# DavidRother/cooking_zoo

Hardware: AMD Instinct MI355X
Metric: env-steps/sec at N parallel envs (1/2/4/8 GPU) + achieved HBM GB/s (higher is better)
Workload: dtype u8/u32 state, f64 obs+reward

## Files before the change

cooking_zoo_amd/csrc/cz_device.h:

```cpp
#pragma once
#include <hip/hip_runtime.h>
#include <stdint.h>
#include <type_traits>

namespace cz {

constexpr int MAX_AGENTS = 4;
constexpr int MAX_NODES = 8;
constexpr int WIDE_NODES = 16;
constexpr int HDR_WORDS = 8;
constexpr int AGENT_WORD0 = HDR_WORDS;
constexpr int RET_WORD0 = HDR_WORDS + MAX_AGENTS;
constexpr int CELL_WORD0 = RET_WORD0 + 2 * MAX_AGENTS;

enum : uint32_t { FLOOR = 0, COUNTER, DELIVERSQUARE, SWITCH, BLOCK, CUTBOARD, BLENDER };
enum : uint32_t { PLATE = 0, ONION, TOMATO, LETTUCE, CARROT, CUCUMBER, BANANA, APPLE, WATERMELON, BREAD };
enum : uint32_t { CELL_TYPE = 7, CELL_READY = 8, CELL_TOGGLE = 16, CELL_ACTIVE = 32, CELL_WALK = 64 };
enum : uint32_t { D_ALIVE = 1u << 24, D_CHOPPED = 2u << 24, D_MASHED = 4u << 24, D_FREE = 8u << 24, D_DONE = 6u << 24 };
enum : uint32_t { COND_NONE = 0, COND_CHOPPED, COND_MASHED, COND_NOT_CHOPPED, COND_NOT_MASHED };
enum : uint32_t { W_T = 0, W_MARKS, W_LAYOUT, W_STATUS, W_EPISODE, W_RECIPES, W_POOL, W_MARKS_HI };
enum : uint32_t { ST_DONE = 1, ST_TERM = 2, ST_TRUNC = 4 };
constexpr int LUT_Y0 = 63, LUT_ZERO = 126, LUT_ONE = 127;
constexpr int LUT_NDONE0 = 128, LUT_CH0 = 132, LUT_MA0 = 136, LUT_CF0 = 140, LUT_OR0 = 144;
enum : uint32_t { SU_EPISODES = 0, SU_STEPS, SU_LENSUM, SU_TRUNC, SU_TERM, SU_COMPLETED0, SU_LAST_LENGTH = 9, SU_LAST_EPISODE, SU_LAST_FLAGS,
// ... 14 lines not shown
    union {
        uint8_t *codes;
        float *obs32;
    };
    uint32_t *stat_u;
    double *stat_f;
    int64_t env_id_base;
    uint64_t seed;
    double recipe_reward, recipe_penalty, node_reward, time_penalty_step;
    double reward_idle;
    const double *lut;
    int32_t N, A, W, H, D, F, RW, scheme, max_steps, end_all, R, auto_reset, L;
    int32_t T;
    uint32_t step0;
    int32_t dyn0_off, dyn1_off;
    int32_t wt;
    int32_t walk_touches;
    int32_t wide;
#ifdef CZ_PROFILE
    unsigned long long *stamps;
#endif
#ifdef CZ_TIMELINE
    unsigned long long *timeline;
#endif
};
#if !defined(CZ_TIMELINE) && !defined(CZ_PROFILE)
static_assert(sizeof(Params) <= 264 && sizeof(Params) % 8 == 0, "argument block: see the note above");
#endif

struct LeanParams {
    const uint32_t *recipes;
    const uint32_t *lay_desc;
    int32_t L, F;
    int32_t max_steps;
    uint32_t settings;
    double reward_idle;
    double *rewards;
    uint8_t *term, *trunc;
    double *obs;
    int32_t auto_reset;
    int32_t reserved;
    uint32_t *stat_u;
    double *stat_f;
    const uint32_t *lay_init;
    int64_t env_id_base;
    double node_reward, recipe_reward, recipe_penalty, time_penalty_step;
#ifdef CZ_PROFILE
    unsigned long long *stamps;
#endif
#ifdef CZ_TIMELINE
    unsigned long long *timeline;
#endif
};
constexpr int LEADING_SCALAR_BYTES = 56;
#if !defined(CZ_TIMELINE) && !defined(CZ_PROFILE)
static_assert(LEADING_SCALAR_BYTES + sizeof(LeanParams) <= 4 * 64, "the lean argument block: four 64-byte lines with the leading scalars");
#endif
static_assert(LEADING_SCALAR_BYTES + offsetof(LeanParams, obs) + sizeof(double *) == 2 * 64, "the common path's fields end the second line");
struct LeanView : LeanParams {
    uint32_t *state;
    const int32_t *actions;
    const double *lut;
    int32_t N, RW, W, H, D, dyn0_off, dyn1_off;
    static constexpr int32_t wide = 0, wt = 1, T = 1;
    static constexpr uint32_t step0 = 0u;
    static constexpr uint64_t seed = 0u;
    static constexpr uint8_t *codes = nullptr;
    int32_t R, end_all, walk_touches;
    LeanView() = default;
    __host__ __device__ explicit LeanView(const LeanParams &b)
        : LeanParams(b), R((int32_t)(b.settings & 0xFFu)), end_all((int32_t)((b.settings >> 8) & 1u)), walk_touches((int32_t)((b.settings >> 16) & 1u)) {}
};
template <int R_, int END_ALL, int WALK_TOUCHES>
struct LeanViewFixed : LeanView {
    static_assert(R_ >= 1 && R_ <= 4 && (END_ALL | 1) == 1 && (WALK_TOUCHES | 1) == 1, "no such handle");
    static constexpr int32_t R = R_, end_all = END_ALL, walk_touches = WALK_TOUCHES;
    using LeanView::LeanView;
};
template <class PB> using block_of = std::conditional_t<std::is_base_of<LeanParams, PB>::value, LeanParams, Params>;

#ifndef CZ_PRIO
#define CZ_PRIO 1
#endif
#if CZ_PRIO
#define CZ_SETPRIO(p) __builtin_amdgcn_s_setprio(p)
#else
#define CZ_SETPRIO(p) do { } while (0)
#endif
__device__ __forceinline__ uint32_t rfl(uint32_t v) { return __builtin_amdgcn_readfirstlane(v); }
__device__ __forceinline__ uint32_t rdl(uint32_t v, int l) { return __builtin_amdgcn_readlane(v, l); }
__device__ __forceinline__ uint64_t ballot(bool p) { return __builtin_amdgcn_ballot_w64(p); }
__device__ __forceinline__ bool lanes(uint64_t m) { return __builtin_amdgcn_inverse_ballot_w64(m); }
extern "C" __device__ uint32_t __cz_writelane(uint32_t, uint32_t, uint32_t) __asm("llvm.amdgcn.writelane.i32");
__device__ __forceinline__ uint32_t wrl(uint32_t value, int lane, uint32_t into) { return __cz_writelane(value, (uint32_t)lane, into); }

__host__ __device__ inline uint32_t action_hash(uint64_t seed, int64_t env_global, int agent, uint32_t step, uint32_t n) {
    uint32_t x = (uint32_t)seed ^ ((uint32_t)(seed >> 32) * 0x9E3779B1u);
    x ^= (uint32_t)env_global * 0x85EBCA6Bu + (uint32_t)((uint64_t)env_global >> 32) * 0x27D4EB2Fu;
    x ^= ((uint32_t)agent + 1u) * 0xC2B2AE35u;
    x ^= (step + 1u) * 0x165667B1u;
    x ^= x >> 16; x *= 0x7FEB352Du; x ^= x >> 15; x *= 0x846CA68Bu; x ^= x >> 16;
    x += step * 0x9E3779B9u;
    x ^= x >> 16; x *= 0x7FEB352Du; x ^= x >> 15; x *= 0x846CA68Bu; x ^= x >> 16;
    return (uint32_t)(((uint64_t)x * (uint64_t)n) >> 32);
}
__host__ __device__ inline uint32_t next_layout(int64_t env_global, uint32_t episode, uint32_t pool_word, uint32_t n_layouts,
                                                uint32_t groups = 1u, uint32_t active = 0u) {
    uint32_t base = pool_word & 0xFFFFu, count = pool_word >> 16;
    if (count == 0) { base = 0; count = n_layouts; }
    if (groups > 1u) { count /= groups; base += active * count; }
    return base + (uint32_t)(((uint64_t)env_global + (uint64_t)episode * 7919u) % count);
}
constexpr int LAY_CTL_WORDS = 16;
enum : uint32_t { LC_GROUPS = 0, LC_ACTIVE = 1 };

struct SpawnCfg {
    uint64_t seed;
    double despawn_rate, respawn_rate;
    uint32_t grace_period;
    uint32_t stride;
    const uint8_t *areas;
    const uint8_t *level_of_layout;
    uint32_t *exhausted;
};
static_assert(sizeof(SpawnCfg) == 56, "layout of the block behind Params::lut");
constexpr uint32_t SPAWN_CFG_OFFSET = 256 * 8 + 64 * 4;
constexpr uint32_t COORD_TABLE_OFFSET = SPAWN_CFG_OFFSET + 56, ROWSEL_TABLE_OFFSET = COORD_TABLE_OFFSET + 1024 * 4;
constexpr uint32_t LUT_BLOCK_BYTES = ROWSEL_TABLE_OFFSET + 64 * 4;
constexpr int SPAWN_GONE0 = 8, SPAWN_GRACE0 = 12;
__host__ __device__ inline uint32_t spawn_grace_bits(uint32_t grace_period, int n_agents) { return grace_period <= 31u ? 5u : 20u / (uint32_t)n_agents; }
__host__ __device__ inline uint32_t spawn_max_grace(int n_agents) { const uint32_t b = 20u / (uint32_t)n_agents; return b > 5u ? (1u << b) - 1u : 31u; }
__host__ __device__ inline uint32_t spawn_initial_status(uint32_t packed_grace, int n_agents) {
    const uint32_t grace = packed_grace & 0xFFFFFFu, bits = packed_grace >> 24;
    uint32_t st = 0;
    for (int a = 0; a < n_agents; ++a) st |= grace << (SPAWN_GRACE0 + bits * a);
    return st;
}

enum : uint32_t { HDR_LAYOUT = 1u, HDR_RECIPE = 2u, HDR_POOL = 4u };
__host__ __device__ inline uint32_t record_header_faults(uint32_t layout, uint32_t recipes, uint32_t pool, uint32_t L, int R, uint32_t n_recipes) {
    uint32_t faults = layout < L ? 0u : HDR_LAYOUT;
    for (int k = 0; k < R; ++k)
        if (((recipes >> (8 * k)) & 0xFFu) >= n_recipes) faults |= HDR_RECIPE;
    const uint32_t base = pool & 0xFFFFu, count = pool >> 16;
    if (count && base + count > L) faults |= HDR_POOL;
    return faults;
}
__host__ __device__ inline bool slot_dead_but_tagged(uint32_t d0, uint32_t d1) { return !(d0 & D_ALIVE) && (d1 & 0xFFu); }

__host__ __device__ inline uint64_t spawn_mix(uint64_t x) {
    x = (x ^ (x >> 30)) * 0xBF58476D1CE4E5B9ull;
    x = (x ^ (x >> 27)) * 0x94D049BB133111EBull;
    return x ^ (x >> 31);
}
__host__ __device__ inline double spawn_uniform(uint64_t seed, uint64_t env_global, uint64_t step_key, uint32_t agent, uint32_t draw) {
    uint64_t k = spawn_mix(seed + 0x9E3779B97F4A7C15ull * env_global);
    k = spawn_mix(k ^ (step_key * 0xD1B54A32D192ED03ull));
    k = spawn_mix(k ^ ((uint64_t)agent << 32) ^ (uint64_t)draw);
    return (double)(k >> 11) * (1.0 / 9007199254740992.0);
}

template <int N>
struct Mask {
    uint64_t w[N];
    __device__ __forceinline__ bool any() const {
        uint64_t o = 0;
// ... 250 lines not shown
                const OM fr = dyn & m_d0_any(e, D_FREE);
                const int grab = fr.any() ? fr.first() : dyn.last();
                if (direct.test(grab)) {
                    me.h = grab;
                    touch(dt, slot_d0(e, grab));
                    move_obj(e, cx, grab, me.xy);
                }
            }
        } else {
            dt.interacted = 1;
            attempt_merge(e, cx, me, dyn, lxy, c, sv, dt);
        }
    }

    static __device__ __forceinline__ void pick_up_special(E &e, const Ctx &cx, Me &me, const OM &dyn, Dirty &dt) {
        if (me.h >= 0 || !dyn.any()) return;
        const OM plates = dyn & m_d0(e, 0xFF0000u, PLATE << 16);
        if (plates.count() != 1) return;
        const int p = plates.first();
        const OM cm = content_of(e, p);
        const int cnt = cm.count();
        if (cnt == 0) return;
        const OM lastm = cm & m_d1(e, 0xFF00u, (uint32_t)(cnt - 1) << 8);
        const int s = lastm.first();
#pragma unroll
        for (int k = 0; k < OPL; ++k) {
            const bool mine = (cx.lane + 64 * k) == s;
            e.d1[k] = mine ? 0u : e.d1[k];
        }
        me.h = s;
        touch(dt, slot_d0(e, s));
        move_obj(e, cx, s, me.xy);
        dt.interacted = 1;
    }

    static __device__ __forceinline__ void execute(E &e, const Ctx &cx, uint32_t lxy, int c, uint32_t sv, const OM &dyn, Dirty &dt) {
        const uint32_t ty = sv & CELL_TYPE;
        if (ty == CUTBOARD) {
            if (!(sv & CELL_READY)) return;
            const OM fresh = dyn & outside_plates(e) & m_d0(e, D_CHOPPED, 0u);
            const int f = fresh.first();
            if (f < 0) return;
            const uint32_t fw = slot_d0(e, f);
            slot_or(e, cx, f, D_CHOPPED);
            if ((fw & 0xFF0000u) == (BREAD << 16)) {
                const OM spare = m_d0(e, D_ALIVE | 0xFF0000u, BREAD << 16);
                const int n = spare.first();
#pragma unroll
                for (int k = 0; k < OPL; ++k) {
                    const bool mine = (cx.lane + 64 * k) == n;
                    e.d0[k] = mine ? (lxy | (BREAD << 16) | D_ALIVE | D_CHOPPED | D_FREE) : e.d0[k];
                    e.d1[k] = mine ? 0u : e.d1[k];
                }
            }
            cell_update(e, cx, c, CELL_READY, 0, dt);
            touch_change(dt, fw, fw | D_CHOPPED);
            dt.interacted = 1;
        } else if (ty == BLENDER) {
            if (sv & CELL_READY) cell_update(e, cx, c, 0, CELL_TOGGLE, dt);
        }
    }

    static __device__ __forceinline__ bool cell_bit(const CM &m, uint32_t c) {
        if constexpr (CPL == 1) {
            return ((m.w[0] >> (c & 63u)) & 1ull) != 0ull;
        } else {
            uint32_t hit = 0u;
#pragma unroll
            for (int k = 0; k < CPL; ++k) {
                const uint32_t lo = (uint32_t)m.w[k], hi = (uint32_t)(m.w[k] >> 32);
                const uint32_t half = (c & 32u) ? hi : lo;
                hit |= ((c >> 6) == (uint32_t)k) ? (half >> (c & 31u)) : 0u;
            }
            return (hit & 1u) != 0u;
        }
    }
    template <int CTRL>
    static __device__ __forceinline__ uint32_t quad(uint32_t v) {
        return (uint32_t)__builtin_amdgcn_mov_dpp((int)v, CTRL, 0xF, 0xF, true);
    }

    struct Pre { uint64_t inter; uint32_t txy, c, act; };

    static __device__ __forceinline__ void perform_agent_actions(E &e, const Ctx &cx, uint32_t act_raw, Dirty &dt) {
        const Pre pre = agents_walk(e, cx, act_raw, dt);
        agents_interact(e, cx, pre, dt);
    }

    static __device__ __forceinline__ Pre agents_walk(E &e, const Ctx &cx, uint32_t act_raw, Dirty &dt) {
        const uint32_t W = (uint32_t)cx.W, H = (uint32_t)cx.H;
        const uint64_t present_m = ~(uint64_t)((e.status >> SPAWN_GONE0) & 0xFu);
        const uint32_t agw = e.agw;
        const uint32_t x = agw & 0xFFu, y = (agw >> 8) & 0xFFu, xy = agw & 0xFFFFu;
        const uint64_t agent_m = ballot((int32_t)act_raw >= 0) & ((1ull << NA) - 1ull) & present_m;
        const uint32_t act0 = lanes(agent_m) ? (act_raw & 7u) : 0u;
        const uint32_t sh = 2u * act0;
        const uint32_t tx = x + ((DX_TABLE >> sh) & 3u) - 1u, ty = y + ((DY_TABLE >> sh) & 3u) - 1u;
        uint32_t ag = lanes(ballot(act0 - 1u < 4u)) ? ((agw & 0xFF00FFFFu) | (act0 << 16)) : agw;
        const uint64_t inb_m = ballot(tx < W) & ballot(ty < H);
        const uint32_t own = __umul24(y, W) + x;
        uint32_t txy = lanes(inb_m) ? (tx | (ty << 8)) : xy;
        uint32_t c = lanes(inb_m) ? (__umul24(ty, W) + tx) : own;
        uint64_t moving_m = ballot(act0 != 0u) & inb_m;
        CM walk_set, switch_set;
#pragma unroll
        for (int k = 0; k < CPL; ++k) {
            walk_set.w[k] = ballot(walkable(e.cell[k]));
            switch_set.w[k] = ballot((e.cell[k] & CELL_TYPE) == SWITCH);
        }
        const uint64_t wk_m = ballot(cell_bit(walk_set, c));
        if (NA > 1) {
            const uint32_t endxy = lanes(wk_m) ? txy : xy;
            const uint32_t exy = lanes(agent_m) ? endxy : (0xFFFF0000u | (uint32_t)cx.lane);
            uint64_t clash_m;
            if (NA == 2) {
                clash_m = ballot(exy == quad<0xB1>(exy));
            } else {
                const uint32_t r1 = quad<0x39>(exy), r2 = quad<0x4E>(exy), r3 = quad<0x93>(exy);
                clash_m = ballot(exy == r1) | ballot(exy == r2) | ballot(exy == r3);
            }
            const uint64_t cancel_m = clash_m & wk_m & moving_m;
            txy = lanes(cancel_m) ? xy : txy;
            c = lanes(cancel_m) ? own : c;
            moving_m &= ~cancel_m;
        }
        const uint32_t act = lanes(moving_m) ? act0 : 0u;
        uint64_t walks_m = agent_m & wk_m;
        if (SCHEME != 3) walks_m &= ballot(act - 1u < 4u);
        ag = lanes(walks_m) ? ((ag & 0xFFFF0000u) | txy) : ag;
        e.agw = ag;
        uint64_t drag = walks_m & moving_m & ballot(ag > 0x00FFFFFFu);
        if (drag) {
            dt.moved = 1;
            do {
                const int a = __builtin_ctzll(drag);
                drag &= drag - 1;
                const uint32_t A = rdl(e.agw, a);
                move_obj(e, cx, (int)(A >> 24) - 1, A & 0xFFFFu);
            } while (drag);
        }
        uint64_t press = walks_m & ballot(cell_bit(switch_set, c));
        if (press) {
            dt.pressed = 1;
            do {
                const int a = __builtin_ctzll(press);
                press &= press - 1;
                cell_update(e, cx, (int)rdl(c, a), 0, CELL_ACTIVE, dt);
            } while (press);
        }
        return Pre{agent_m & ~walks_m & (SCHEME == 3 ? moving_m : ballot(act >= 5u)), txy, c, act};
    }

    static __device__ __forceinline__ void agents_interact(E &e, const Ctx &cx, const Pre &pre, Dirty &dt) {
        const uint32_t W = (uint32_t)cx.W, H = (uint32_t)cx.H;
        const uint32_t txy = pre.txy, c = pre.c, act = pre.act;
        uint64_t inter = pre.inter;
        if (inter & (inter - 1)) CZ_SETPRIO(2);
        else if (inter) CZ_SETPRIO(1);
#ifndef CZ_INTER_UNROLL
#define CZ_INTER_UNROLL 0
#endif
#if CZ_INTER_UNROLL
#pragma unroll
        for (int a = 0; a < NA; ++a) {
            if (!((inter >> a) & 1ull)) continue;
#else
        while (inter) {
            const int a = __builtin_ctzll(inter);
            inter &= inter - 1;
#endif
            const uint32_t A = rdl(e.agw, a);
            Me me{A & 0xFFFFu, (int)(A >> 24) - 1};
            uint32_t fxy;
            int fc;
            bool ok = true;
            if (SCHEME == 3) {
                fxy = rdl(txy, a);
                fc = (int)rdl(c, a);
            } else {
                const uint32_t o = (A >> 16) & 0xFFu;
                const uint32_t fx = (A & 0xFFu) + ((DX_TABLE >> (2u * o)) & 3u) - 1u;
                const uint32_t fy = ((A >> 8) & 0xFFu) + ((DY_TABLE >> (2u * o)) & 3u) - 1u;
                ok = fx < W && fy < H;
                fxy = fx | (fy << 8);
                fc = (int)(fy * W + fx);
            }
            const uint32_t sv = ok ? cell_at(e, fc) : 0u;
            if (ok && holds_objects(sv & CELL_TYPE)) {
                const OM dyn = m_d0(e, D_ALIVE | 0xFFFFu, D_ALIVE | fxy);
                if (SCHEME == 3) {
                    bool exec = false;
                    if ((sv & CELL_TYPE) >= CUTBOARD) exec = (dyn & m_d0(e, D_DONE, 0u)).any();
                    if (exec) execute(e, cx, fxy, fc, sv, dyn, dt);
                    else primary(e, cx, me, fxy, fc, sv, dyn, dt);
                } else {
                    const int ac = (int)rdl(act, a);
                    if (ac == 5) primary(e, cx, me, fxy, fc, sv, dyn, dt);
                    else if (ac == 6) pick_up_special(e, cx, me, dyn, dt);
                    else execute(e, cx, fxy, fc, sv, dyn, dt);
                }
                e.agw = wrl((A & 0x00FFFFFFu) | ((uint32_t)((me.h + 1) & 0xFF) << 24), a, e.agw);
            }
        }
    }

    static __device__ __forceinline__ uint32_t handle_agent_spawn(E &e, const Ctx &cx, const SpawnCfg *cfg_generic, int64_t env_global) {
        typedef const __attribute__((address_space(4))) SpawnCfg *kcfg;
        const kcfg cfg = (kcfg)cfg_generic;
        const uint64_t seed = cfg->seed, key = ((uint64_t)e.episode << 32) | (uint64_t)e.t;
        const double despawn_rate = cfg->despawn_rate, respawn_rate = cfg->respawn_rate;
        uint32_t st = e.status, gone = 0u;
        const uint32_t packed_grace = cfg->grace_period, gbits = packed_grace >> 24, gmask = (1u << gbits) - 1u;
#pragma unroll
        for (int a = 0; a < NA; ++a) {
            const uint32_t gsh = (uint32_t)SPAWN_GRACE0 + gbits * (uint32_t)a;
            if ((st >> gsh) & gmask) { st -= 1u << gsh; continue; }
            const bool despawned = (st >> (SPAWN_GONE0 + a)) & 1u;
            if (!despawned) {
                const int n_active = NA - __popc((st >> SPAWN_GONE0) & 0xFu);
                if (n_active > 1 && spawn_uniform(seed, (uint64_t)env_global, key, (uint32_t)a, 0u) < despawn_rate) {
                    if ((rdl(e.agw, a) >> 24) == 0u) {
                        st |= 1u << (SPAWN_GONE0 + a);
                        gone |= 1u << a;
                    }
                }
            } else if (spawn_uniform(seed, (uint64_t)env_global, key, (uint32_t)a, 1u) < respawn_rate) {
                st = (st & ~(1u << (SPAWN_GONE0 + a))) | ((packed_grace & 0xFFFFFFu) << gsh);
                typedef const __attribute__((address_space(4))) uint8_t *kbytes;
                const uint32_t stride = cfg->stride, level = ((kbytes)cfg->level_of_layout)[e.layout];
                const kbytes blk = (kbytes)cfg->areas + (size_t)(level * (uint32_t)MAX_AGENTS + (uint32_t)a) * (4u + 2u * stride);
                const uint32_t nx = (uint32_t)blk[0] | ((uint32_t)blk[1] << 8), ny = (uint32_t)blk[2] | ((uint32_t)blk[3] << 8);
                bool placed = false;
#pragma nounroll
                for (uint32_t k = 0; k < 1001u; ++k) {
                    const uint32_t ix = (uint32_t)(spawn_uniform(seed, (uint64_t)env_global, key, (uint32_t)a, 2u + 2u * k) * (double)nx);
                    const uint32_t iy = (uint32_t)(spawn_uniform(seed, (uint64_t)env_global, key, (uint32_t)a, 3u + 2u * k) * (double)ny);
                    const uint32_t x = blk[4u + ix], y = blk[4u + stride + iy];
                    if (x >= (uint32_t)cx.W || y >= (uint32_t)cx.H) continue;
                    if ((cell_at(e, (int)(y * (uint32_t)cx.W + x)) & CELL_TYPE) != FLOOR) continue;
// ... 305 lines not shown
```

cooking_zoo_amd/csrc/cz_kernels.h:

```cpp
#pragma once
#include "cz_device.h"
#include <type_traits>

namespace cz {

#ifdef CZ_PROFILE
#define CZ_STAMP(i)                                                                                    \
    do {                                                                                               \
        unsigned long long _t;                                                                         \
        __builtin_amdgcn_sched_barrier(0);                                                             \
        asm volatile("s_memrealtime %0\n\ts_waitcnt lgkmcnt(0)" : "=s"(_t)::"memory");                 \
        __builtin_amdgcn_sched_barrier(0);                                                             \
        if (lane == 0 && P.stamps) P.stamps[(size_t)env * 16 + (i)] = _t;                               \
    } while (0)
#elif defined(CZ_MARKERS)
#define CZ_STAMP(i) asm volatile("; CZ_MARK " #i)
#else
#define CZ_STAMP(i) do { } while (0)
#endif

typedef const __attribute__((address_space(4))) Params *KParams;
struct StepArgsMirror { uint32_t *a; const int32_t *b; const double *c; int32_t i[8]; Params p; };
struct LeanArgsMirror { uint32_t *a; const int32_t *b; const double *c; int32_t i[8]; LeanParams p; };
static_assert(offsetof(LeanArgsMirror, p) == LEADING_SCALAR_BYTES && offsetof(StepArgsMirror, p) == LEADING_SCALAR_BYTES, "leading scalars");
template <class B> constexpr unsigned block_offset() {
    return std::is_same<B, LeanParams>::value ? (unsigned)offsetof(LeanArgsMirror, p) : (unsigned)offsetof(StepArgsMirror, p);
}
template <class B = Params>
__device__ __forceinline__ const __attribute__((address_space(4))) B *late_params(unsigned offset) {
    const __attribute__((address_space(4))) char *k =
        (const __attribute__((address_space(4))) char *)__builtin_amdgcn_kernarg_segment_ptr();
    asm volatile("" : "+s"(k));
    return reinterpret_cast<const __attribute__((address_space(4))) B *>(k + offset);
}
#define CZ_LATE_STEP() late_params<typename V::Block>(block_offset<typename V::Block>())

enum StepMode : int {
    STEP = 0,
    ROLLOUT = 1,
    ROLLOUT_ACTIONS = 2,
    STEP_CODES = 3,
    ROLLOUT_CODES = 4,
    ROLLOUT_CODES_ONLY = 5,
    STEP_F32 = 6,
    ROLLOUT_F32 = 7,
    ROLLOUT_ACTIONS_F32 = 8,
};
template <int MODE, bool LEAN = false>
struct StepTraits {
    static_assert(MODE >= STEP && MODE <= ROLLOUT_ACTIONS_F32 && (!LEAN || MODE == STEP), "no such variant");
    static constexpr bool fused = MODE == ROLLOUT || MODE == ROLLOUT_ACTIONS || MODE == ROLLOUT_CODES || MODE == ROLLOUT_CODES_ONLY ||
                                  MODE == ROLLOUT_F32 || MODE == ROLLOUT_ACTIONS_F32;
    static constexpr bool ext_actions = MODE == ROLLOUT_ACTIONS || MODE == ROLLOUT_ACTIONS_F32;
    static constexpr bool codes = MODE == STEP_CODES || MODE == ROLLOUT_CODES || MODE == ROLLOUT_CODES_ONLY;
    static constexpr bool codes_only = MODE == ROLLOUT_CODES_ONLY;
    static constexpr bool f32 = MODE == STEP_F32 || MODE == ROLLOUT_F32 || MODE == ROLLOUT_ACTIONS_F32;
    static constexpr bool f64 = !codes_only && !f32;
#ifndef CZ_ROLLOUT_F32_HOLD
#define CZ_ROLLOUT_F32_HOLD 1
#endif
    static constexpr bool desc_held = (codes || f32) && (!fused || codes_only || (f32 && CZ_ROLLOUT_F32_HOLD != 0));
    static constexpr bool desc_per_step = (codes || f32) && fused && !desc_held;
    static constexpr bool lean = LEAN;
    using Block = std::conditional_t<LEAN, LeanParams, Params>;
    using View = std::conditional_t<LEAN, LeanView, Params>;
};
template <int R, int END_ALL, int WALK_TOUCHES>
struct LeanCfgTraits : StepTraits<STEP, true> {
    using View = LeanViewFixed<R, END_ALL, WALK_TOUCHES>;
};

template <int CPL>
struct Img {
    static constexpr bool HUGE = CPL > 4;
    static constexpr int OBJ0 = 0, CELL0 = HUGE ? 1536 : 768, AG0 = CELL0 + (HUGE ? 4096 : 1024), ZERO = AG0 + 32, HALFWORDS = ZERO + 8;
};
constexpr int LUT_ABSENT = 255, LUT_SIZE = 256;
#ifndef CZ_ENVS_PER_WG
#define CZ_ENVS_PER_WG 8
#endif
constexpr int ENVS_PER_WG = CZ_ENVS_PER_WG;
template <int CPL> constexpr int envs_per_wg() { return CPL > 4 ? 4 : ENVS_PER_WG; }
constexpr int OBS_PAIRS = 3;
constexpr int OBS_CHUNK = 2 * OBS_PAIRS;

template <int CPL>
struct Lds {
    int32_t sub[MAX_AGENTS][16];
    uint16_t img[Img<CPL>::HALFWORDS];
    uint64_t locs[CPL <= 4 ? 64 * CPL + 8 : WIDE_NODES * CPL];
};

template <class T>
__device__ __forceinline__ T ldg(const void *sbase, uint32_t voff) {
    return *reinterpret_cast<const T *>(reinterpret_cast<const char *>(sbase) + voff);
}
template <class T>
__device__ __forceinline__ void stg(void *sbase, uint32_t voff, T v) {
    *reinterpret_cast<T *>(reinterpret_cast<char *>(sbase) + voff) = v;
}
template <class T>
__device__ __forceinline__ void stg_wt(void *sbase, uint32_t voff, T v) {
    __hip_atomic_store(reinterpret_cast<T *>(reinterpret_cast<char *>(sbase) + voff), v, __ATOMIC_RELAXED, __HIP_MEMORY_SCOPE_AGENT);
}

typedef double double2_t __attribute__((ext_vector_type(2)));
typedef uint32_t uint2_t __attribute__((ext_vector_type(2)));
typedef uint32_t uint4_t __attribute__((ext_vector_type(4)));

template <int OPL, int CPL, int NA, bool LEAN = false, class PB>
__device__ __forceinline__ void load_env(const PB &P, Env<OPL, CPL, NA> &e, const Ctx &cx, const uint32_t *__restrict__ rec) {
    const uint32_t lane = (uint32_t)cx.lane;
    uint32_t hw[HDR_WORDS];
    {
        typedef const __attribute__((address_space(4))) uint32_t *kconst_u32;
        const kconst_u32 hp = (kconst_u32)rec;
#pragma unroll
        for (int i = 0; i < HDR_WORDS; ++i) hw[i] = hp[i];
    }
    const uint32_t aw = ldg<uint32_t>(rec, (AGENT_WORD0 + (lane & 3u)) * 4u);
#pragma unroll
    for (int k = 0; k < CPL; ++k) {
        const uint32_t c = lane + 64u * k;
        const uint32_t v = ldg<uint8_t>(rec, CELL_WORD0 * 4u + min(c, (uint32_t)cx.C - 1u));
        e.cell[k] = (c < (uint32_t)cx.C) ? v : 0u;
    }
#pragma unroll
    for (int k = 0; k < OPL; ++k) {
        const uint32_t s = lane + 64u * k, sc = min(s, (uint32_t)cx.D - 1u);
        const uint32_t a = ldg<uint32_t>(rec, ((uint32_t)P.dyn0_off + sc) * 4u), b = ldg<uint32_t>(rec, ((uint32_t)P.dyn1_off + sc) * 4u);
        e.d0[k] = (s < (uint32_t)cx.D) ? a : 0u;
        e.d1[k] = (s < (uint32_t)cx.D) ? b : 0u;
    }
    __builtin_amdgcn_sched_barrier(0);
    e.t = hw[W_T]; e.marks = hw[W_MARKS]; e.layout = hw[W_LAYOUT]; e.status = hw[W_STATUS];
    e.episode = hw[W_EPISODE]; e.recipes = hw[W_RECIPES]; e.pool = hw[W_POOL];
    e.marks_hi = !LEAN && P.wide ? hw[W_MARKS_HI] : 0u;
    e.agw = (lane < (uint32_t)NA) ? aw : 0u;
}

template <int OPL, int CPL, int NA, class PB>
__device__ __forceinline__ void store_env(const PB &P, const Env<OPL, CPL, NA> &e, const Ctx &cx, uint32_t *__restrict__ rec,
                                          bool cells_dirty, bool objs_dirty, bool header_dirty = true) {
    const uint32_t lane = (uint32_t)cx.lane;
    if (header_dirty) {
        uint32_t h = 0;
        h = wrl(e.t, W_T, h);
        h = wrl(e.marks, W_MARKS, h);
        h = wrl(e.layout, W_LAYOUT, h);
        h = wrl(e.status, W_STATUS, h);
        h = wrl(e.episode, W_EPISODE, h);
        h = wrl(e.recipes, W_RECIPES, h);
        h = wrl(e.pool, W_POOL, h);
        h = wrl(e.marks_hi, W_MARKS_HI, h);
        if (lane < (uint32_t)HDR_WORDS) stg<uint32_t>(rec, lane * 4u, h);
    } else if (lane == 0u) {
        stg<uint32_t>(rec, W_T * 4u, e.t);
    }
    if (lane < (uint32_t)MAX_AGENTS) stg<uint32_t>(rec, (AGENT_WORD0 + lane) * 4u, e.agw);
    if (cells_dirty) {
#pragma unroll
        for (int k = 0; k < CPL; ++k) {
            const uint32_t c = lane + 64u * k;
            if (c < (uint32_t)cx.C) stg<uint8_t>(rec, CELL_WORD0 * 4u + c, (uint8_t)e.cell[k]);
        }
    }
    if (objs_dirty) {
#pragma unroll
        for (int k = 0; k < OPL; ++k) {
            const uint32_t s = lane + 64u * k;
            if (s < (uint32_t)cx.D) {
                stg<uint32_t>(rec, ((uint32_t)P.dyn0_off + s) * 4u, e.d0[k]);
                stg<uint32_t>(rec, ((uint32_t)P.dyn1_off + s) * 4u, e.d1[k]);
            }
        }
    }
}

template <class PB>
__device__ __forceinline__ uint32_t load_row_selector(const PB &P, int lane) { return ldg<uint32_t>(P.lut, ROWSEL_TABLE_OFFSET + (uint32_t)lane * 4u); }
template <class PB>
__device__ __forceinline__ uint32_t load_recipe_rows(const PB &P, uint32_t recipes, uint32_t sel) {
    const uint32_t id = (recipes >> (sel & 0xFFu)) & 0xFFu;
    return ldg<uint32_t>(P.recipes, __umul24(id, (1u + MAX_NODES) * 4u) + (sel >> 8));
}
template <class PB>
__device__ __forceinline__ uint32_t load_recipe_rows(const PB &P, uint32_t recipes, int lane) {
    return load_recipe_rows(P, recipes, load_row_selector(P, lane));
}

template <int OPL, int CPL, int NA, bool LEAN = false, class PB>
__device__ __forceinline__ void all_marks(const PB &P, Env<OPL, CPL, NA> &e, const Ctx &cx, uint32_t rowv, Lds<CPL> &s) {
    uint32_t lo = 0, hi = 0;
    if (!LEAN && __builtin_expect(P.wide != 0, 0)) {
#pragma nounroll
        for (int r = 0; r < P.R; ++r) {
            const uint32_t id = (e.recipes >> (8 * r)) & 0xFFu;
            const uint32_t m = Ops<OPL, CPL, NA, 3>::recipe_marks_wide(e, cx, P.recipes + (size_t)id * (1 + 2 * WIDE_NODES), s.locs);
            if (r < 2) lo |= m << (16 * r); else hi |= m << (16 * (r - 2));
        }
    } else {
        if constexpr (CPL <= 4) {
            lo = Ops<OPL, CPL, NA, 3>::recipe_marks_cells(e, cx, rowv, 0xFu, P.R, s.locs);
        } else {
#pragma nounroll
            for (int r = 0; r < P.R; ++r) lo |= Ops<OPL, CPL, NA, 3>::recipe_marks(e, cx, rowv, 9 * r, s.locs) << (8 * r);
        }
    }
    e.marks = lo; e.marks_hi = hi;
}

template <class PB>
__device__ __forceinline__ uint32_t load_submask(const PB &P, int lane) { return ldg<uint32_t>(P.lut, (uint32_t)(LUT_SIZE * 8 + lane * 4)); }

__device__ __forceinline__ void init_lut(const Params &P, double *lut, int tid, int nthreads) {
    for (int i = tid; i < LUT_SIZE; i += nthreads) lut[i] = ldg<double>(P.lut, (uint32_t)i * 8u);
}

template <int CPL> struct CoordWords { uint32_t w[CPL]; };
template <int CPL, class PB>
__device__ __forceinline__ CoordWords<CPL> load_coord_words(const PB &P, int lane) {
    CoordWords<CPL> cw;
#pragma unroll
    for (int k = 0; k < CPL; ++k) cw.w[k] = ldg<uint32_t>(P.lut, COORD_TABLE_OFFSET + (uint32_t)(lane + 64 * k) * 4u);
    return cw;
}
template <int CPL>
__device__ __forceinline__ void init_lds(const Ctx &cx, Lds<CPL> &s, const CoordWords<CPL> &cw) {
    const int lane = cx.lane;
    s.img[Img<CPL>::ZERO] = (uint16_t)(LUT_ABSENT * 8);
    uint32_t *img32 = reinterpret_cast<uint32_t *>(s.img);
#pragma unroll
    for (int k = 0; k < CPL; ++k) {
        const uint32_t c = (uint32_t)(lane + 64 * k);
        img32[(Img<CPL>::CELL0 >> 1) + 2 * c] = cw.w[k];
    }
}
template <int CPL, class PB>
__device__ __forceinline__ void init_lds(const PB &P, const Ctx &cx, Lds<CPL> &s) {
    const int lane = cx.lane;
    s.img[Img<CPL>::ZERO] = (uint16_t)(LUT_ABSENT * 8);
    uint32_t *img32 = reinterpret_cast<uint32_t *>(s.img);
#pragma unroll
    for (int k = 0; k < CPL; ++k) {
        const uint32_t c = (uint32_t)(lane + 64 * k);
        img32[(Img<CPL>::CELL0 >> 1) + 2 * c] = ldg<uint32_t>(P.lut, COORD_TABLE_OFFSET + c * 4u);
    }
}

template <class PB>
__device__ __forceinline__ void load_desc(const PB &P, uint32_t layout, int chunk, int lane, uint32_t (&dsc)[OBS_CHUNK]) {
    const auto rs = __builtin_amdgcn_make_buffer_rsrc(const_cast<uint32_t *>(P.lay_desc), 0, P.L * P.F * 4, 0x00020000);
    const uint32_t row = layout * (uint32_t)P.F * 4u;
#pragma unroll
    for (int i = 0; i < OBS_CHUNK / 2; ++i) {
        const uint32_t f = (uint32_t)(chunk * (OBS_CHUNK / 2) + i) * 128u + 2u * (uint32_t)lane;
        const uint2_t d = __builtin_bit_cast(uint2_t, __builtin_amdgcn_raw_buffer_load_b64(rs, f * 4u, row, 0));
        dsc[2 * i] = d.x; dsc[2 * i + 1] = d.y;
// ... 147 lines not shown
        if (chunk > 0) load_desc(P, e.layout, chunk, cx.lane, dsc);
        uint32_t b[OBS_CHUNK];
        int sb[NA][OBS_CHUNK];
        double2_t v[NA][OBS_PAIRS];
#pragma unroll
        for (int j = 0; j < OBS_CHUNK; ++j) b[j] = *reinterpret_cast<const uint16_t *>(imgb + (dsc[j] & 0xFFFFu));
#pragma unroll
        for (int a = 0; a < NA; ++a)
#pragma unroll
            for (int j = 0; j < OBS_CHUNK; ++j) sb[a][j] = *reinterpret_cast<const int32_t *>(subb + 64 * a + (dsc[j] >> 16));
#pragma unroll
        for (int a = 0; a < NA; ++a)
#pragma unroll
            for (int i = 0; i < OBS_PAIRS; ++i) {
                v[a][i].x = *reinterpret_cast<const double *>(lutb + ((int)b[2 * i] - sb[a][2 * i]));
                v[a][i].y = *reinterpret_cast<const double *>(lutb + ((int)b[2 * i + 1] - sb[a][2 * i + 1]));
            }
        const uint32_t f0b = (uint32_t)(chunk * OBS_PAIRS * 128 + 2 * cx.lane) * 8u;
#define CZ_OBS_WRITE_ROWS(AUX)                                                                                               \
    _Pragma("unroll") for (int i = 0; i < OBS_PAIRS; ++i)                                                                    \
        _Pragma("unroll") for (int a = 0; a < NA; ++a)                                                                       \
            __builtin_amdgcn_raw_buffer_store_b128(__builtin_bit_cast(uint4_t, v[a][i]), rs[a], f0b + (uint32_t)i * 1024u, 0, AUX)
        if (wt == 1u) { CZ_OBS_WRITE_ROWS(16); }
        else if (wt == 2u) { CZ_OBS_WRITE_ROWS(2); }
        else { CZ_OBS_WRITE_ROWS(0); }
#undef CZ_OBS_WRITE_ROWS
    }
    if (!LEAN && P.F > 128 * OBS_PAIRS) load_desc(P, e.layout, 0, cx.lane, dsc);
    __builtin_amdgcn_wave_barrier();
}

struct StepOut {
    double myrew;
    uint32_t term, trunc;
    bool stepped, finished;
    bool header;
    uint32_t gone;
#ifdef CZ_TIMELINE
    uint32_t dbg;
#endif
};

#define CZ_RARE(hint, x) ((hint) ? __builtin_expect(!!(x), 0) : !!(x))
template <int OPL, int CPL, int NA, int SCHEME, bool FUSED, bool LEAN, class PB>
__device__ __forceinline__ void step_env(const PB &P, unsigned kp_off, Env<OPL, CPL, NA> &e, const Ctx &cx, uint32_t acts,
                                         int64_t env_global, uint32_t &rowv, Lds<CPL> &lds, uint32_t (&dsc)[OBS_CHUNK], Dirty &dt, StepOut &o) {
    using O = Ops<OPL, CPL, NA, SCHEME>;
    o.myrew = 0.0;
    o.term = 0; o.trunc = 0; o.stepped = false; o.finished = false; o.header = false; o.gone = 0u;
#ifdef CZ_TIMELINE
    o.dbg = 0u;
#endif
    const bool spawning = !LEAN && (P.auto_reset & 2) != 0;
    const SpawnCfg *const spawn_cfg = reinterpret_cast<const SpawnCfg *>(reinterpret_cast<const char *>(P.lut) + SPAWN_CFG_OFFSET);
    if (CZ_RARE(FUSED, (e.status & ST_DONE) != 0u)) {
        o.header = true;
        if (P.auto_reset & 1) {
            e.episode += 1;
            const uint32_t *const lay0 = late_params<block_of<PB>>(kp_off)->lay_init;
            typedef const __attribute__((address_space(4))) uint32_t *kconst_u32;
            const kconst_u32 ctl = (kconst_u32)(lay0 - LAY_CTL_WORDS);
            uint32_t lay = next_layout(env_global, e.episode, e.pool, (uint32_t)P.L, ctl[LC_GROUPS], ctl[LC_ACTIVE]);
            uint32_t recipes = e.recipes, episode = e.episode, pool = e.pool;
            load_env<OPL, CPL, NA, LEAN>(P, e, cx, lay0 + (size_t)lay * P.RW);
            e.t = 0; e.layout = lay; e.status = 0; e.episode = episode; e.recipes = recipes; e.pool = pool;
            if (spawning) {
                typedef const __attribute__((address_space(4))) SpawnCfg *kcfg;
                e.status = spawn_initial_status(((kcfg)spawn_cfg)->grace_period, NA);
            }
            all_marks<OPL, CPL, NA, LEAN>(P, e, cx, rowv, lds);
            if (LEAN || P.obs) load_desc(P, lay, 0, cx.lane, dsc);
            dt.cells = 1; dt.touched = 1; dt.interacted = 1;
        } else {
            o.term = (e.status & ST_TERM) ? 1u : 0u;
            o.trunc = (e.status & ST_TRUNC) ? 1u : 0u;
        }
        return;
    }
    o.stepped = true;
    e.t += 1;
#if defined(CZ_PROFILE)
    const int lane = cx.lane; const long long env = env_global - P.env_id_base;
#endif
    O::perform_agent_actions(e, cx, acts, dt);
    CZ_STAMP(2);
    O::progress_and_link(e, cx, dt);
    if (spawning) {
        o.gone = O::handle_agent_spawn(e, cx, spawn_cfg, env_global);
        o.header = true;
    }
    CZ_STAMP(3);
    const bool truncated = (int)e.t >= P.max_steps;
    const uint32_t before = e.marks;
    uint32_t after = before;
    o.myrew = cx.lane < NA ? P.reward_idle : 0.0;
    if (dt.moved & (uint32_t)P.walk_touches) { dt.touched = 1; dt.kinds = ~0ull; }
    if (dt.kinds & 0xFull) dt.kinds = ~0ull;
    bool done = false;
    if (!LEAN && __builtin_expect(P.wide != 0, 0)) {
        if (dt.touched) {
            uint32_t lo = 0, hi = 0;
#pragma nounroll
            for (int r = 0; r < P.R; ++r) {
                const uint32_t id = (e.recipes >> (8 * r)) & 0xFFu;
                const uint32_t *row = P.recipes + (size_t)id * (1 + 2 * WIDE_NODES);
                const uint32_t mb_r = ((r < 2 ? e.marks : e.marks_hi) >> (16 * (r & 1))) & 0xFFFFu;
                const uint32_t ma = O::recipe_marks_wide(e, cx, row, lds.locs);
                if (r < 2) lo |= ma << (16 * r); else hi |= ma << (16 * (r - 2));
                if (ma != mb_r) {
                    uint32_t countmask = 0;
                    const int n = (int)(rfl(row[0]) & 0xFFu);
#pragma nounroll
                    for (int j = 0; j < n; ++j) countmask |= ((rfl(row[1 + 2 * j]) >> 8) & 1u) << j;
                    const int goals_before = __popc(~mb_r & countmask), goals_after = __popc(~ma & countmask);
                    const bool completed = ma & 1, completion_before = mb_r & 1;
                    const bool malus = !completed && completion_before, bonus = completed && !completion_before;
                    const auto kp = late_params<block_of<PB>>(kp_off);
                    double x = 0.0;
                    x += (double)(goals_before - goals_after) * kp->node_reward;
                    x += (bonus ? 1.0 : 0.0) * kp->recipe_reward;
                    x += (malus ? 1.0 : 0.0) * kp->recipe_penalty;
                    x += kp->time_penalty_step;
                    if (cx.lane == r && r < NA) o.myrew = x;
                }
            }
            o.header |= lo != e.marks || hi != e.marks_hi;
            e.marks = lo; e.marks_hi = hi;
        }
        const uint32_t rlo = e.marks & (P.R >= 2 ? 0x00010001u : 0x00000001u);
        const uint32_t rhi = P.R >= 3 ? (e.marks_hi & (P.R >= 4 ? 0x00010001u : 0x00000001u)) : 0u;
        const int n_roots = __popc(rlo) + __popc(rhi);
        done = P.end_all ? (n_roots == P.R) : (n_roots != 0);
    } else {
        if (dt.touched) {
            const uint32_t nw = rowv, lane_u = (uint32_t)cx.lane;
            const uint32_t r_of = (lane_u * 57u) >> 9;
            const uint32_t seen = (uint32_t)(dt.kinds >> ((nw >> 14) & 0x3Cu)) & ((nw >> 24) & 0xFu);
            const uint32_t kids = nw & 0xFFu, mb = (before >> (8u * (r_of & 3u))) & 0xFFu;
            constexpr uint64_t NODE_LANES = 0x1FEull | (0x1FEull << 9) | (0x1FEull << 18) | (0x1FEull << 27);
            const bool rel = (nw & 0x2000u) != 0u && seen != 0u, sens = kids != 0u && (mb & kids) == kids;
            const auto reward_of = [&](int r, uint32_t mb_r, uint32_t ma) {
                const uint32_t countmask = (uint32_t)((ballot((nw & 0x100u) != 0u) >> (9 * r + 1)) & 0xFFull);
                const int goals_before = __popc(~mb_r & countmask), goals_after = __popc(~ma & countmask);
                const bool completed = ma & 1, completion_before = mb_r & 1;
                const bool malus = !completed && completion_before, bonus = completed && !completion_before;
                const auto kp = late_params<block_of<PB>>(kp_off);
                double x = 0.0;
                x += (double)(goals_before - goals_after) * kp->node_reward;
                x += (bonus ? 1.0 : 0.0) * kp->recipe_reward;
                x += (malus ? 1.0 : 0.0) * kp->recipe_penalty;
                x += kp->time_penalty_step;
                if (cx.lane == r && r < NA) o.myrew = x;
            };
            CZ_STAMP(8);
            if constexpr (CPL <= 4) {
                const uint32_t flags = (rel ? 1u : 0u) | (sens ? 16u : 0u);
                const uint32_t any = O::wave_or(lanes(NODE_LANES) ? (flags << (r_of & 3u)) : 0u);
                const uint32_t which = any & (dt.statechg != 0u ? 0xFu : (any >> 4)) & ((1u << P.R) - 1u);
                if (which) {
                    CZ_SETPRIO(3);
#ifdef CZ_TIMELINE
                    o.dbg |= 2u;
#endif
                    const uint32_t fresh = O::recipe_marks_cells(e, cx, rowv, which, P.R, lds.locs);
                    CZ_STAMP(9);
                    const uint32_t bytes = ((which * 0x204081u) & 0x01010101u) * 0xFFu;
                    after = (before & ~bytes) | (fresh & bytes);
// ... 102 lines not shown
    bool cells_dirty = false, objs_dirty = false, header_dirty = V::fused;
    bool img_objs = true, img_cells = true;
    float *const lutf = reinterpret_cast<float *>(lut);
    if (V::f32) { if (threadIdx.x < (unsigned)LUT_SIZE) lutf[threadIdx.x] = (float)lutv; }
    else if (threadIdx.x < (unsigned)LUT_SIZE) lut[threadIdx.x] = lutv;
    __syncthreads();
    if (env_raw >= P.N) return;
    CZ_STAMP(1);
    CodesPrefetch cpre;
    cpre.layout = e.layout;
    if (V::desc_held) {
#pragma unroll
        for (int r = 0; r < CODES_PREFETCH; ++r) cpre.d[r] = load_desc4(P, e.layout, 256u * r + 4u * (uint32_t)lane);
    }

    const int T = V::fused ? P.T : 1;
#ifdef CZ_TIMELINE
    uint32_t tl_dbg = 0u;
#endif
    const uint32_t act_lane = ((uint32_t)env * (uint32_t)NA + (uint32_t)min(lane, NA - 1)) * 4u;
    if (V::ext_actions) av = ldg<int>(e_actions, act_lane);
#pragma nounroll
    for (int t = 0; t < T; ++t) {
        typename V::View Pt;
        if constexpr (V::fused) {
            static_assert(sizeof(Params) % 8 == 0, "copied as 64-bit words");
            typedef uint64_t __attribute__((may_alias)) word_t;
            const __attribute__((address_space(4))) word_t *src = (const __attribute__((address_space(4))) word_t *)CZ_LATE_STEP();
            word_t *dst = reinterpret_cast<word_t *>(&Pt);
#pragma unroll
            for (unsigned i = 0; i < sizeof(Params) / 8; ++i) dst[i] = src[i];
            Pt.state = e_state; Pt.actions = e_actions; Pt.lut = e_lut; Pt.N = e_N; Pt.RW = e_RW; Pt.W = e_W; Pt.H = e_H; Pt.D = e_D;
            Pt.dyn0_off = e_dyn0; Pt.dyn1_off = e_dyn1;
        } else {
            Pt = P;
        }
        if (V::desc_per_step) {
            cpre.layout = e.layout;
#pragma unroll
            for (int r = 0; r < CODES_PREFETCH; ++r) cpre.d[r] = load_desc4(Pt, e.layout, 256u * r + 4u * (uint32_t)lane);
        }
        uint32_t acts;
        if (!V::fused) acts = (uint32_t)av;
        else if (V::ext_actions) {
            acts = (uint32_t)av;
            av = ldg<int>(e_actions, act_lane + (uint32_t)min(t + 1, T - 1) * ((uint32_t)Pt.N * (uint32_t)NA * 4u));
        } else acts = action_hash(Pt.seed, env_global, lane & 3, Pt.step0 + (uint32_t)t, SCHEME == 3 ? 5u : 8u);
        Dirty dt{};
        StepOut o;
        step_env<OPL, CPL, NA, SCHEME, V::fused, V::lean>(Pt, block_offset<typename V::Block>(), e, cx, acts, env_global, rowv, lds, dsc, dt, o);
#ifdef CZ_TIMELINE
        tl_dbg |= o.dbg;
#endif
        CZ_STAMP(4);
        cells_dirty |= dt.cells != 0;
        objs_dirty |= (dt.touched | dt.interacted | dt.moved) != 0;
        header_dirty |= o.header;
        const double myrew = o.myrew;
        if (o.stepped) ret += myrew;
        const auto kp = CZ_LATE_STEP();
        uint32_t su_old = 0u;
        double sf_old = 0.0, ret_done = 0.0;
        if (CZ_RARE(V::fused, o.finished)) {
            const uint32_t *su = kp->stat_u + (size_t)env * SU_WORDS;
            const double *sf = kp->stat_f + (size_t)env * SF_WORDS;
            su_old = ldg<uint32_t>(su, ((uint32_t)lane & 15u) * 4u);
            sf_old = ldg<double>(sf, (uint32_t)(SF_SUM0 + ((uint32_t)lane & 3u)) * 8u);
            ret_done = ret;
            ret = 0.0;
        }
        const bool in_place = V::ext_actions && !V::f32 && (Pt.step0 & 1u) != 0u;
        const size_t row = V::fused ? ((size_t)(in_place ? 0 : t) * Pt.N + env) : (size_t)env;
        if (V::codes || V::f32) {
            if (CZ_RARE(V::fused, cpre.layout != e.layout)) {
                cpre.layout = e.layout;
#pragma unroll
                for (int r = 0; r < CODES_PREFETCH; ++r) cpre.d[r] = load_desc4(Pt, e.layout, 256u * r + 4u * (uint32_t)lane);
            }
#pragma unroll
            for (int r = 0; r < CODES_PREFETCH; ++r) asm volatile("" :: "v"(cpre.d[r]));
        }
        {
            const uint32_t oidx = (uint32_t)row * (uint32_t)NA + (uint32_t)lane;
            double *const rewards = kp->rewards;
            uint8_t *const term = kp->term, *const trunc = kp->trunc;
            if (lane < NA) {
                if (!V::fused || rewards) stg<double>(rewards, oidx * 8u, myrew);
                if (!V::fused || term) stg<uint8_t>(term, oidx, (uint8_t)o.term);
                if (!V::fused || trunc) {
                    stg<uint8_t>(trunc, oidx, (uint8_t)o.trunc);
                    if (o.gone && ((o.gone >> lane) & 1u)) stg<uint8_t>(trunc, oidx, (uint8_t)1);
                }
            }
        }
        if constexpr (!V::fused && !V::lean) {
            uint32_t *const marks_out = kp->marks_out;
            if (marks_out && lane < 2) stg<uint32_t>(marks_out, (2u * (uint32_t)env + (uint32_t)lane) * 4u, lane == 0 ? e.marks : e.marks_hi);
        }
        CZ_STAMP(5);
        img_objs |= (dt.touched | dt.moved) != 0;
        img_cells |= dt.cells != 0;
        if constexpr (V::f32) {
            float *const obs_row = Pt.obs32 + (uint64_t)(uint32_t)row * (uint64_t)(uint32_t)(NA * Pt.F);
            build_image<OPL, CPL, NA>(Pt, e, cx, lds, submask, img_objs, img_cells);
            write_rows_f32<OPL, CPL, NA>(Pt, e, cx, lds, lutf, obs_row, &cpre);
            if (V::fused) { img_objs = false; img_cells = false; }
        } else if (V::lean || Pt.obs || V::codes) {
            uint8_t *const codes = V::codes ? Pt.codes + (uint64_t)(uint32_t)row * (uint64_t)(uint32_t)(NA * codes_pitch(Pt.F)) : nullptr;
            double *const obs_row = V::f64 && Pt.obs ? Pt.obs + (uint64_t)(uint32_t)row * (uint64_t)(uint32_t)(NA * Pt.F) : nullptr;
            observe<OPL, CPL, NA, V::f64, V::lean>(Pt, e, cx, lds, lut, dsc, submask, obs_row, img_objs, img_cells, codes, V::codes ? &cpre : nullptr);
            img_objs = false; img_cells = false;
        }
        if (CZ_RARE(V::fused, o.finished)) {
            uint32_t *su = kp->stat_u + (size_t)env * SU_WORDS;
            double *sf = kp->stat_f + (size_t)env * SF_WORDS;
            const uint32_t a_of = (uint32_t)lane - SU_COMPLETED0;
            const uint32_t root = !V::lean && Pt.wide ? (((a_of < 2u ? e.marks : e.marks_hi) >> (16u * (a_of & 1u))) & 1u) : ((e.marks >> (8u * (a_of & 3u))) & 1u);
            const uint32_t inc = lane == (int)SU_EPISODES ? 1u : lane == (int)SU_LENSUM ? e.t : lane == (int)SU_TRUNC ? (uint32_t)o.trunc
                                 : lane == (int)SU_TERM ? (uint32_t)o.term : a_of < (uint32_t)NA ? root : 0u;
            if (lane < (int)SU_COMPLETED0 + NA && lane != (int)SU_STEPS) stg<uint32_t>(su, (uint32_t)lane * 4u, su_old + inc);
            if (lane < NA) stg<double>(sf, (uint32_t)(SF_SUM0 + lane) * 8u, sf_old + ret_done);
            const uint32_t roots = (uint32_t)(ballot(a_of < (uint32_t)NA && root != 0u) >> SU_COMPLETED0) & 0xFu;
            const uint32_t last = lane == (int)SU_LAST_LENGTH ? e.t : lane == (int)SU_LAST_EPISODE ? e.episode
                                  : (uint32_t)o.term | ((uint32_t)o.trunc << 1) | (roots << 4);
            if (lane >= (int)SU_LAST_LENGTH && lane <= (int)SU_LAST_FLAGS) stg<uint32_t>(su, (uint32_t)lane * 4u, last);
            if (lane < NA) stg<double>(sf, (uint32_t)(SF_LAST0 + lane) * 8u, ret_done);
        }
        CZ_STAMP(6);
    }
    store_env(P, e, cx, rec, cells_dirty, objs_dirty, header_dirty);
    if (lane < NA) stg<double>(retp, (uint32_t)lane * 8u, ret);
    CZ_STAMP(7);
#ifdef CZ_TIMELINE
    {
        const uint64_t tl_out = wall_clock64();
        const uint32_t hw_id = __builtin_amdgcn_s_getreg(4 | (31 << 11)), xcc = __builtin_amdgcn_s_getreg(20 | (31 << 11));
        unsigned long long *const tl = CZ_LATE_STEP()->timeline;
        if (tl && lane == 0) {
            typedef unsigned long long ull2 __attribute__((ext_vector_type(2)));
            ull2 v;
            v.x = (tl_in & 0xFFFFFFFFull) | ((unsigned long long)(hw_id & 0xFFFFu) << 32) | ((unsigned long long)tl_dbg << 48);
            v.y = (tl_out & 0xFFFFFFFFull) | ((unsigned long long)(xcc & 15u) << 32) | (((tl_seen - tl_in) & 0xFFFFFFFull) << 36);
            *reinterpret_cast<ull2 *>(tl + 2 * (size_t)env) = v;
        }
    }
#endif
}

#ifdef CZ_STEP_MIN_WPE
#define CZ_STEP_ATTR __attribute__((amdgpu_waves_per_eu((!StepTraits<FUSED>::fused && OPL <= 2) ? CZ_STEP_MIN_WPE : 1)))
#else
#define CZ_STEP_ATTR
#endif
template <int OPL, int CPL, int NA, int SCHEME, int FUSED >
__global__ __launch_bounds__(64 * envs_per_wg<CPL>()) CZ_STEP_ATTR void k_step(uint32_t *e_state, const int32_t *e_actions, const double *e_lut, int32_t e_N,
                                                          int32_t e_RW, int32_t e_W, int32_t e_H, int32_t e_D, int32_t e_dyn0,
                                                          int32_t e_dyn1, const Params P0) {
    step_kernel<OPL, CPL, NA, SCHEME, StepTraits<FUSED>>(e_state, e_actions, e_lut, e_N, e_RW, e_W, e_H, e_D, e_dyn0, e_dyn1, P0);
}
template <int OPL, int CPL, int NA, int SCHEME>
__global__ __launch_bounds__(64 * envs_per_wg<CPL>()) void k_step_lean(uint32_t *e_state, const int32_t *e_actions, const double *e_lut, int32_t e_N,
                                                                       int32_t e_RW, int32_t e_W, int32_t e_H, int32_t e_D, int32_t e_dyn0,
                                                                       int32_t e_dyn1, const LeanParams P0) {
    step_kernel<OPL, CPL, NA, SCHEME, StepTraits<STEP, true>>(e_state, e_actions, e_lut, e_N, e_RW, e_W, e_H, e_D, e_dyn0, e_dyn1, P0);
}
template <int OPL, int CPL, int NA, int SCHEME, int R, int END_ALL, int WALK_TOUCHES>
__global__ __launch_bounds__(64 * envs_per_wg<CPL>()) void k_step_lean_cfg(uint32_t *e_state, const int32_t *e_actions, const double *e_lut, int32_t e_N,
                                                                           int32_t e_RW, int32_t e_W, int32_t e_H, int32_t e_D, int32_t e_dyn0,
                                                                           int32_t e_dyn1, const LeanParams P0) {
    step_kernel<OPL, CPL, NA, SCHEME, LeanCfgTraits<R, END_ALL, WALK_TOUCHES>>(e_state, e_actions, e_lut, e_N, e_RW, e_W, e_H, e_D, e_dyn0, e_dyn1, P0);
}
__device__ __forceinline__ void init_lut_f32(const Params &P, float *lutf, int lane) {
    for (int i = lane; i < LUT_SIZE; i += 64) lutf[i] = (float)ldg<double>(P.lut, (uint32_t)i * 8u);
}
template <class T>
__device__ __forceinline__ T *row_of(T *base, size_t i, size_t pitch) { return base ? base + i * pitch : nullptr; }
template <int OPL, int CPL, int NA>
__device__ __forceinline__ void write_forms(const Params &P, const Env<OPL, CPL, NA> &e, const Ctx &cx, Lds<CPL> &lds, double *lut, float *lutf,
                                            double *obs, float *obs32, uint8_t *codes, size_t row) {
    const uint32_t submask = load_submask(P, cx.lane);
    if (obs || codes) {
        if (obs) init_lut(P, lut, cx.lane, 64);
        uint32_t dsc[OBS_CHUNK];
        load_desc(P, e.layout, 0, cx.lane, dsc);
        observe(P, e, cx, lds, lut, dsc, submask, row_of(obs, row, (size_t)NA * P.F), true, true, row_of(codes, row, (size_t)NA * codes_pitch(P.F)));
    }
    if (obs32) {
        init_lut_f32(P, lutf, cx.lane);
        if (!(obs || codes)) build_image<OPL, CPL, NA>(P, e, cx, lds, submask, true, true);
        write_rows_f32<OPL, CPL, NA>(P, e, cx, lds, lutf, obs32 + row * NA * P.F, nullptr);
    }
}
template <int OPL, int CPL, int NA>
__device__ __forceinline__ void begin_episode(const Params &P, Env<OPL, CPL, NA> &e, const Ctx &cx, Lds<CPL> &lds, uint32_t *rec, uint32_t lay,
                                              uint32_t episode, uint32_t recipes, uint32_t pool) {
    load_env(P, e, cx, P.lay_init + (size_t)lay * P.RW);
    e.t = 0; e.layout = lay; e.status = 0; e.episode = episode; e.recipes = recipes; e.pool = pool;
    if (P.auto_reset & 2)
        e.status = spawn_initial_status(rfl(reinterpret_cast<const SpawnCfg *>(reinterpret_cast<const char *>(P.lut) + SPAWN_CFG_OFFSET)->grace_period), NA);
    uint32_t rowv = load_recipe_rows(P, e.recipes, cx.lane);
    all_marks(P, e, cx, rowv, lds);
    store_env(P, e, cx, rec, true, true);
    if (cx.lane < MAX_AGENTS) reinterpret_cast<double *>(rec + RET_WORD0)[cx.lane] = 0.0;
}

template <int OPL, int CPL, int NA>
__global__ __launch_bounds__(64) void k_reset(const Params P, int64_t env_begin, const int32_t *__restrict__ layout_ids,
                                              const uint32_t *__restrict__ recipe_words, const uint32_t *__restrict__ pool_words,
                                              double *obs_out) {
    __shared__ Lds<CPL> lds;
    __shared__ double lut[LUT_SIZE];
    const int i = blockIdx.x;
    Ctx cx{P.W, P.H, P.D, P.W * P.H, (int)threadIdx.x};
    init_lds<CPL>(P, cx, lds);
// ... 255 lines not shown
```

Baseline: 765.1 million.

## Trim lean step path: skip idle interact, assume presence, ranged buffer writeback

```diff
diff --git a/cooking_zoo_amd/csrc/cz_device.h b/cooking_zoo_amd/csrc/cz_device.h
--- a/cooking_zoo_amd/csrc/cz_device.h
+++ b/cooking_zoo_amd/csrc/cz_device.h
@@ -120,6 +120,9 @@
 #ifndef CZ_PRIO
 #define CZ_PRIO 1
 #endif
+#ifndef CZ_LEAN_TRIM
+#define CZ_LEAN_TRIM 15
+#endif
 #if CZ_PRIO
 #define CZ_SETPRIO(p) __builtin_amdgcn_s_setprio(p)
 #else
@@ -536,14 +539,16 @@
 
     struct Pre { uint64_t inter; uint32_t txy, c, act; };
 
+    template <bool LEAN = false>
     static __device__ __forceinline__ void perform_agent_actions(E &e, const Ctx &cx, uint32_t act_raw, Dirty &dt) {
-        const Pre pre = agents_walk(e, cx, act_raw, dt);
-        agents_interact(e, cx, pre, dt);
-    }
-
+        const Pre pre = agents_walk<LEAN>(e, cx, act_raw, dt);
+        agents_interact<LEAN>(e, cx, pre, dt);
+    }
+
+    template <bool LEAN = false>
     static __device__ __forceinline__ Pre agents_walk(E &e, const Ctx &cx, uint32_t act_raw, Dirty &dt) {
         const uint32_t W = (uint32_t)cx.W, H = (uint32_t)cx.H;
-        const uint64_t present_m = ~(uint64_t)((e.status >> SPAWN_GONE0) & 0xFu);
+        const uint64_t present_m = LEAN && (CZ_LEAN_TRIM & 2) ? ~0ull : ~(uint64_t)((e.status >> SPAWN_GONE0) & 0xFu);
         const uint32_t agw = e.agw;
         const uint32_t x = agw & 0xFFu, y = (agw >> 8) & 0xFFu, xy = agw & 0xFFFFu;
         const uint64_t agent_m = ballot((int32_t)act_raw >= 0) & ((1ull << NA) - 1ull) & present_m;
@@ -605,10 +610,12 @@
         return Pre{agent_m & ~walks_m & (SCHEME == 3 ? moving_m : ballot(act >= 5u)), txy, c, act};
     }
 
+    template <bool LEAN = false>
     static __device__ __forceinline__ void agents_interact(E &e, const Ctx &cx, const Pre &pre, Dirty &dt) {
         const uint32_t W = (uint32_t)cx.W, H = (uint32_t)cx.H;
         const uint32_t txy = pre.txy, c = pre.c, act = pre.act;
         uint64_t inter = pre.inter;
+        if (LEAN && (CZ_LEAN_TRIM & 1) && !inter) return;
         if (inter & (inter - 1)) CZ_SETPRIO(2);
         else if (inter) CZ_SETPRIO(1);
 #ifndef CZ_INTER_UNROLL
diff --git a/cooking_zoo_amd/csrc/cz_kernels.h b/cooking_zoo_amd/csrc/cz_kernels.h
--- a/cooking_zoo_amd/csrc/cz_kernels.h
+++ b/cooking_zoo_amd/csrc/cz_kernels.h
@@ -62,6 +62,8 @@
     static constexpr bool desc_held = (codes || f32) && (!fused || codes_only || (f32 && CZ_ROLLOUT_F32_HOLD != 0));
     static constexpr bool desc_per_step = (codes || f32) && fused && !desc_held;
     static constexpr bool lean = LEAN;
+    static constexpr bool ranged_writeback = LEAN && (CZ_LEAN_TRIM & 8) != 0;
+    static constexpr bool block_outputs = LEAN && (CZ_LEAN_TRIM & 4) != 0;
     using Block = std::conditional_t<LEAN, LeanParams, Params>;
     using View = std::conditional_t<LEAN, LeanView, Params>;
 };
@@ -174,6 +176,48 @@
                 stg<uint32_t>(rec, ((uint32_t)P.dyn1_off + s) * 4u, e.d1[k]);
             }
         }
+    }
+}
+
+template <int OPL, int CPL, int NA, class PB>
+__device__ __forceinline__ void store_env_ranged(const PB &P, const Env<OPL, CPL, NA> &e, const Ctx &cx, uint32_t *__restrict__ rec,
+                                                 bool cells_dirty, bool objs_dirty, bool header_dirty, double ret) {
+    static_assert(W_T == 0 && NA <= MAX_AGENTS, "lane MAX_AGENTS carries the step counter");
+    constexpr uint32_t NOWHERE = 0x40000000u;
+    const uint32_t lane = (uint32_t)cx.lane;
+    const auto rs = __builtin_amdgcn_make_buffer_rsrc(rec, 0, P.RW * 4, 0x00020000);
+    {
+        const bool t_lane = lane == (uint32_t)MAX_AGENTS;
+        const uint32_t off = t_lane ? (uint32_t)W_T * 4u : (AGENT_WORD0 + lane) * 4u;
+        __builtin_amdgcn_raw_buffer_store_b32(t_lane ? e.t : e.agw, rs, lane <= (uint32_t)MAX_AGENTS ? off : NOWHERE, 0, 0);
+    }
+    constexpr bool BRANCHES = (CZ_LEAN_TRIM & 16) != 0;
+    const uint32_t c_end = BRANCHES || cells_dirty ? (uint32_t)cx.C : 0u, d_end = BRANCHES || objs_dirty ? (uint32_t)cx.D : 0u;
+    if (!BRANCHES || cells_dirty)
+#pragma unroll
+    for (int k = 0; k < CPL; ++k) {
+        const uint32_t c = lane + 64u * k;
+        __builtin_amdgcn_raw_buffer_store_b8((uint8_t)e.cell[k], rs, c < c_end ? CELL_WORD0 * 4u + c : NOWHERE, 0, 0);
+    }
+    if (!BRANCHES || objs_dirty)
+#pragma unroll
+    for (int k = 0; k < OPL; ++k) {
+        const uint32_t s = lane + 64u * k;
+        __builtin_amdgcn_raw_buffer_store_b32(e.d0[k], rs, s < d_end ? ((uint32_t)P.dyn0_off + s) * 4u : NOWHERE, 0, 0);
+        __builtin_amdgcn_raw_buffer_store_b32(e.d1[k], rs, s < d_end ? ((uint32_t)P.dyn1_off + s) * 4u : NOWHERE, 0, 0);
+    }
+    __builtin_amdgcn_raw_buffer_store_b64(__builtin_bit_cast(uint2_t, ret), rs, lane < (uint32_t)NA ? RET_WORD0 * 4u + lane * 8u : NOWHERE, 0, 0);
+    if (header_dirty) {
+        uint32_t h = 0;
+        h = wrl(e.t, W_T, h);
+        h = wrl(e.marks, W_MARKS, h);
+        h = wrl(e.layout, W_LAYOUT, h);
+        h = wrl(e.status, W_STATUS, h);
+        h = wrl(e.episode, W_EPISODE, h);
+        h = wrl(e.recipes, W_RECIPES, h);
+        h = wrl(e.pool, W_POOL, h);
+        h = wrl(e.marks_hi, W_MARKS_HI, h);
+        __builtin_amdgcn_raw_buffer_store_b32(h, rs, lane < (uint32_t)HDR_WORDS ? lane * 4u : NOWHERE, 0, 0);
     }
 }
 
@@ -487,7 +531,7 @@
 #if defined(CZ_PROFILE)
     const int lane = cx.lane; const long long env = env_global - P.env_id_base;
 #endif
-    O::perform_agent_actions(e, cx, acts, dt);
+    O::template perform_agent_actions<LEAN>(e, cx, acts, dt);
     CZ_STAMP(2);
     O::progress_and_link(e, cx, dt);
     if (spawning) {
@@ -756,8 +800,10 @@
         }
         {
             const uint32_t oidx = (uint32_t)row * (uint32_t)NA + (uint32_t)lane;
-            double *const rewards = kp->rewards;
-            uint8_t *const term = kp->term, *const trunc = kp->trunc;
+            double *rewards;
+            uint8_t *term, *trunc;
+            if constexpr (V::block_outputs) { rewards = Pt.rewards; term = Pt.term; trunc = Pt.trunc; }
+            else { rewards = kp->rewards; term = kp->term; trunc = kp->trunc; }
             if (lane < NA) {
                 if (!V::fused || rewards) stg<double>(rewards, oidx * 8u, myrew);
                 if (!V::fused || term) stg<uint8_t>(term, oidx, (uint8_t)o.term);
@@ -781,7 +827,7 @@
             if (V::fused) { img_objs = false; img_cells = false; }
         } else if (V::lean || Pt.obs || V::codes) {
             uint8_t *const codes = V::codes ? Pt.codes + (uint64_t)(uint32_t)row * (uint64_t)(uint32_t)(NA * codes_pitch(Pt.F)) : nullptr;
-            double *const obs_row = V::f64 && Pt.obs ? Pt.obs + (uint64_t)(uint32_t)row * (uint64_t)(uint32_t)(NA * Pt.F) : nullptr;
+            double *const obs_row = V::f64 && (V::block_outputs || Pt.obs) ? Pt.obs + (uint64_t)(uint32_t)row * (uint64_t)(uint32_t)(NA * Pt.F) : nullptr;
             observe<OPL, CPL, NA, V::f64, V::lean>(Pt, e, cx, lds, lut, dsc, submask, obs_row, img_objs, img_cells, codes, V::codes ? &cpre : nullptr);
             img_objs = false; img_cells = false;
         }
@@ -802,8 +848,12 @@
         }
         CZ_STAMP(6);
     }
-    store_env(P, e, cx, rec, cells_dirty, objs_dirty, header_dirty);
-    if (lane < NA) stg<double>(retp, (uint32_t)lane * 8u, ret);
+    if constexpr (V::ranged_writeback) {
+        store_env_ranged(P, e, cx, rec, cells_dirty, objs_dirty, header_dirty, ret);
+    } else {
+        store_env(P, e, cx, rec, cells_dirty, objs_dirty, header_dirty);
+        if (lane < NA) stg<double>(retp, (uint32_t)lane * 8u, ret);
+    }
     CZ_STAMP(7);
 #ifdef CZ_TIMELINE
     {
```

Result: no change. 770.7 million (median of 6 runs) (+0.7%).
